# NVIDIA/cuopt

Measured on NVIDIA H100. Metric: pdlp_iterations_per_sec, higher is better.
Workload: dtype f64

## Files before the change

cuopt_b200/csrc/device_utils.cuh:

```cuda
#pragma once

#include "lp_problem.hpp"

#include <cuda_runtime.h>

#include <chrono>
#include <cstdio>
#include <cstdlib>
#include <mutex>
#include <string>
#include <vector>

namespace cuopt_b200 {

#define CUOPT_CUDA_TRY(call)                                                                              \
  do {                                                                                                    \
    cudaError_t err__ = (call);                                                                           \
    if (err__ != cudaSuccess) {                                                                           \
      cudaGetLastError();                                                                                 \
      throw ::cuopt_b200::lp_error(                                                                       \
        err__ == cudaErrorMemoryAllocation ? ::cuopt_b200::error_type_t::OutOfMemory                      \
                                           : ::cuopt_b200::error_type_t::RuntimeError,                    \
        std::string("CUDA error: ") + cudaGetErrorString(err__) + " at " + __FILE__ + ":" +               \
          std::to_string(__LINE__));                                                                      \
// ... 186 lines not shown
{
#pragma unroll
  for (int o = 16; o > 0; o >>= 1)
    v += __shfl_xor_sync(0xffffffffu, v, o);
  return v;
}
__device__ __forceinline__ double warp_max(double v)
{
#pragma unroll
  for (int o = 16; o > 0; o >>= 1)
    v = fmax(v, __shfl_xor_sync(0xffffffffu, v, o));
  return v;
}

template <bool IsMax = false>
__device__ __forceinline__ double block_reduce(double v, double* scratch)
{
  const int lane = threadIdx.x & 31, wid = threadIdx.x >> 5, nw = (blockDim.x + 31) >> 5;
  v = IsMax ? warp_max(v) : warp_sum(v);
  __syncthreads();
  if (lane == 0) scratch[wid] = v;
  __syncthreads();
  double r = (lane < nw) ? scratch[lane] : 0.0;
  r        = IsMax ? warp_max(r) : warp_sum(r);
  return r;
}

struct l2_policy_t {
  unsigned long long keep, stream;
};
__device__ __forceinline__ l2_policy_t make_l2_policies(int mode)
{
  l2_policy_t p;
  if (mode) {
    asm volatile("createpolicy.fractional.L2::evict_last.b64 %0, 1.0;" : "=l"(p.keep));
    asm volatile("createpolicy.fractional.L2::evict_first.b64 %0, 1.0;" : "=l"(p.stream));
  } else {
    asm volatile("createpolicy.fractional.L2::evict_normal.b64 %0, 1.0;" : "=l"(p.keep));
    p.stream = p.keep;
  }
  return p;
}
__device__ __forceinline__ double ld_l2(const double* p, unsigned long long policy)
{
  double v;
  asm volatile("ld.global.L1::no_allocate.L2::cache_hint.f64 %0, [%1], %2;" : "=d"(v) : "l"(p), "l"(policy));
  return v;
}
__device__ __forceinline__ void st_l2(double* p, double v, unsigned long long policy)
{
  asm volatile("st.global.L2::cache_hint.f64 [%0], %1, %2;" ::"l"(p), "d"(v), "l"(policy) : "memory");
}

__device__ __forceinline__ int ld_stream(const int* p) { return __ldcs(p); }
__device__ __forceinline__ double ld_stream(const double* p) { return __ldcs(p); }

}
```

cuopt_b200/csrc/pdlp_kernels.cuh:

```cuda
#pragma once

#include "device_utils.cuh"
#include "spmv_bicsr.cuh"

#include <math_constants.h>

namespace cuopt_b200 {

constexpr int EW_THREADS  = 256;
static __device__ int g_l2_hints = 1;

struct pdhg_ctl_t {
  double step_size, primal_weight, tau, sigma;
  double pending_weight;
  double sum_weights;
  double interaction, norm_dx2, norm_dy2;
  double reduction_exponent, growth_exponent, primal_smoothing, dual_smoothing;
  int parity;
  int pending_avg;
  int active;
  int valid;
  int k_pdhg;
  int attempts;
  int accepted;
// ... 144 lines not shown
                                                            int n,
                                                            double* __restrict__ xbuf0,
                                                            double* __restrict__ xbuf1,
                                                            const double* __restrict__ aty0,
                                                            const double* __restrict__ aty1,
                                                            const double* __restrict__ c,
                                                            const double* __restrict__ l,
                                                            const double* __restrict__ u,
                                                            double* __restrict__ sum_x,
                                                            double* __restrict__ xbar)
{
  if (!ctl->active) return;
  const int cur           = ctl->parity;
  const double* x         = cur ? xbuf1 : xbuf0;
  double* xn              = cur ? xbuf0 : xbuf1;
  const double* aty       = cur ? aty1 : aty0;
  const double tau        = ctl->tau;
  const bool pending      = ctl->pending_avg != 0;
  const double w          = ctl->pending_weight;
  const int stride        = gridDim.x * blockDim.x;
  const l2_policy_t pol   = make_l2_policies(g_l2_hints);
  for (int j = blockIdx.x * blockDim.x + threadIdx.x; j < n; j += stride) {
    const double xj = x[j];
    if (pending) sum_x[j] = sum_x[j] + w * xj;
    const double gradient = ld_stream(c + j) - aty[j];
    double next           = xj - (tau * gradient);
    next                  = fmax(fmin(next, ld_stream(u + j)), ld_stream(l + j));
    xn[j]                 = next;
    st_l2(xbar + j, next - xj + next, pol.keep);
  }
}

template <bool INIT, int NPRE, bool BCAST = false, int FMT = 0>
__global__ void __launch_bounds__(BICSR_THREADS, bicsr_min_ctas(NPRE)) k_dual_step(pdhg_ctl_t* __restrict__ ctl,
                                                                             bicsr_view_t A,
                                                                             const double* __restrict__ xbar,
                                                                             double* __restrict__ ybuf0,
                                                                             double* __restrict__ ybuf1,
                                                                             const double* __restrict__ lc,
                                                                             const double* __restrict__ uc,
                                                                             double* __restrict__ sum_y,
                                                                             double* __restrict__ part_dy2,
                                                                             const unsigned long long* xbar_flags,
                                                                             int n_xbar_flags,
                                                                             const double* __restrict__ t,
                                                                             peer_ptrs_t y_peers = peer_ptrs_t{},
                                                                             peer_flags_t flags = peer_flags_t{},
                                                                             int world = 1,
                                                                             int rank = 0,
                                                                             const int* __restrict__ send = nullptr,
                                                                             int send_stride = 0)
{
  if (!ctl->active) return;
  __shared__ double rows[BICSR_WARPS][BICSR_SLOTS];
  __shared__ double red[32];
  const unsigned long long epoch = (unsigned long long)ctl->attempts + 1ull;
  if (xbar_flags) peer_wait(xbar_flags, n_xbar_flags, (unsigned long long)ctl->attempts + 1ull);
  const int cur      = ctl->parity;
  const double* y    = cur ? ybuf1 : ybuf0;
  double* yn         = cur ? ybuf0 : ybuf1;
  const double sigma = ctl->sigma;
  const bool pending = ctl->pending_avg != 0;
  const double w     = ctl->pending_weight;
  double dy2         = 0.0;
  const l2_policy_t pol = make_l2_policies(g_l2_hints);
  struct payload_t {
    double y, lc, uc, sum, init;
  };
  auto pre_op = [&](int i) {
    payload_t p;
    p.y    = y[i];
    p.lc   = ld_stream(lc + i);
    p.uc   = ld_stream(uc + i);
    p.sum  = pending ? sum_y[i] : 0.0;
    p.init = INIT ? ld_l2(t + i, pol.stream) : 0.0;
    return p;
  };
  auto row_op = [&](int i, double s, const payload_t& p) {
    if (pending) sum_y[i] = p.sum + w * p.y;
    double next      = p.y - (sigma * s);
    const double low = next + sigma * p.lc;
    const double up  = next + sigma * p.uc;
    next             = fmax(low, fmin(up, 0.0));
    st_l2(yn + i, next, pol.keep);
    if constexpr (BCAST) {
#pragma unroll
      for (int r = 0; r < DIST_MAX_PEERS; ++r)
        if (r < world) {
          const int d = __ldg(send + (size_t)r * send_stride + i);
          if (d >= 0) y_peers.p[r][d] = next;
        }
    }
    const double d   = next - p.y;
    dy2 += d * d;
  };
  spmv_bicsr_rows<payload_t, INIT, NPRE, FMT>(A, xbar, rows[threadIdx.x >> 5], pre_op, row_op, pol.keep);
  const double tot = block_reduce(dy2, red);
  if (threadIdx.x == 0) part_dy2[blockIdx.x] = tot;
  if constexpr (BCAST) peer_signal_grid_done(&ctl->ticket[2], flags, world, DIST_FLAG_Y + rank, epoch, DIST_FLAG_Y_B + rank);
}

template <bool INIT, int NPRE, int FMT = 0>
__global__ void __launch_bounds__(BICSR_THREADS, bicsr_min_ctas(NPRE)) k_transpose_step(pdhg_ctl_t* __restrict__ ctl,
                                                                                  bicsr_view_t AT,
                                                                                  const double* __restrict__ ybuf0,
                                                                                  const double* __restrict__ ybuf1,
                                                                                  const double* __restrict__ xbuf0,
                                                                                  const double* __restrict__ xbuf1,
                                                                                  double* __restrict__ aty0,
                                                                                  double* __restrict__ aty1,
                                                                                  double* __restrict__ parts,
                                                                                  const double* __restrict__ part_dy2,
                                                                                  int n_part_dy2,
                                                                                  const double* __restrict__ t)
{
  if (!ctl->active) return;
  __shared__ double rows[BICSR_WARPS][BICSR_SLOTS];
  __shared__ double red[32];
  const int cur     = ctl->parity;
  const double* yn  = cur ? ybuf0 : ybuf1;
  const double* x   = cur ? xbuf1 : xbuf0;
  const double* xn  = cur ? xbuf0 : xbuf1;
  const double* aty = cur ? aty1 : aty0;
  double* atyn      = cur ? aty0 : aty1;
  double acc[2]     = {0.0, 0.0};
  const l2_policy_t pol = make_l2_policies(g_l2_hints);
  struct payload_t {
    double dx, aty, init;
  };
  auto pre_op = [&](int j) {
    payload_t p;
    p.dx   = ld_l2(xn + j, pol.stream) - ld_l2(x + j, pol.stream);
    p.aty  = ld_l2(aty + j, pol.stream);
    p.init = INIT ? ld_l2(t + j, pol.stream) : 0.0;
    return p;
  };
  auto row_op = [&](int j, double s, const payload_t& p) {
    st_l2(atyn + j, s, pol.stream);
    acc[0] += p.dx * (s - p.aty);
    acc[1] += p.dx * p.dx;
  };
  spmv_bicsr_rows<payload_t, INIT, NPRE, FMT>(AT, yn, rows[threadIdx.x >> 5], pre_op, row_op, pol.keep);

  if (!publish_and_elect<2>(acc, parts, &ctl->ticket[0], red)) return;
  const double interaction = gather_partials(parts, gridDim.x, red);
  const double dx2         = gather_partials(parts + gridDim.x, gridDim.x, red);
  const double dy2         = gather_partials(part_dy2, n_part_dy2, red);
  if (threadIdx.x != 0) return;

  pdhg_step_rule(ctl, interaction, dx2, dy2);
}

template <bool INIT, int NPRE>
__global__ void __launch_bounds__(BICSR_THREADS, bicsr_min_ctas(NPRE)) k_transpose_step_slice(pdhg_ctl_t* __restrict__ ctl,
                                                                                        bicsr_view_t AT,
                                                                                        const double* __restrict__ yfull,
                                                                                        const double* __restrict__ xbuf0,
                                                                                        const double* __restrict__ xbuf1,
                                                                                        double* __restrict__ aty0,
                                                                                        double* __restrict__ aty1,
                                                                                        double* __restrict__ parts,
                                                                                        const double* __restrict__ part_dy2,
                                                                                        int n_part_dy2,
                                                                                        const double* __restrict__ t,
                                                                                        const unsigned long long* wait_flags,
                                                                                        int n_wait,
                                                                                        peer_ptrs_t scal_peers,
                                                                                        peer_flags_t flags,
                                                                                        int world,
                                                                                        int rank)
{
  if (!ctl->active) return;
  __shared__ double rows[BICSR_WARPS][BICSR_SLOTS];
  __shared__ double red[32];
  const unsigned long long epoch = (unsigned long long)ctl->attempts + 1ull;
  if (wait_flags) peer_wait(wait_flags, n_wait, epoch);
  const int cur     = ctl->parity;
  const double* x   = cur ? xbuf1 : xbuf0;
  const double* xn  = cur ? xbuf0 : xbuf1;
  const double* aty = cur ? aty1 : aty0;
  double* atyn      = cur ? aty0 : aty1;
  double acc[2]     = {0.0, 0.0};
  const l2_policy_t pol = make_l2_policies(g_l2_hints);
  struct payload_t {
    double dx, aty, init;
  };
  auto pre_op = [&](int j) {
    payload_t p;
    p.dx   = ld_l2(xn + j, pol.stream) - ld_l2(x + j, pol.stream);
    p.aty  = ld_l2(aty + j, pol.stream);
    p.init = INIT ? ld_l2(t + j, pol.stream) : 0.0;
    return p;
  };
  auto row_op = [&](int j, double s, const payload_t& p) {
    st_l2(atyn + j, s, pol.stream);
    acc[0] += p.dx * (s - p.aty);
    acc[1] += p.dx * p.dx;
  };
  spmv_bicsr_rows<payload_t, INIT, NPRE>(AT, yfull, rows[threadIdx.x >> 5], pre_op, row_op, pol.keep);

  if (!publish_and_elect<2>(acc, parts, &ctl->ticket[0], red)) return;
  const double interaction = gather_partials(parts, gridDim.x, red);
  const double dx2         = gather_partials(parts + gridDim.x, gridDim.x, red);
  const double dy2         = gather_partials(part_dy2, n_part_dy2, red);
  if (threadIdx.x != 0) return;
#pragma unroll
  for (int r = 0; r < DIST_MAX_PEERS; ++r)
    if (r < world) {
      double* o = scal_peers.p[r];
      o[0]      = interaction;
      o[1]      = dx2;
      o[2]      = dy2;
    }
  __threadfence_system();
#pragma unroll
  for (int r = 0; r < DIST_MAX_PEERS; ++r)
    if (r < world) st_release_sys(flags.p[r] + DIST_FLAG_SCALARS + rank, epoch);
}

struct peer_csr_t {
  const int* off[DIST_MAX_PEERS];
  const int* idx[DIST_MAX_PEERS];
  const double* val[DIST_MAX_PEERS];
  int row0[DIST_MAX_PEERS];
};
__global__ void __launch_bounds__(EW_THREADS) k_slice_row_counts(int rows, int j0, peer_csr_t src, int world, int* __restrict__ cnt)
{
  const int stride = gridDim.x * blockDim.x;
  for (int j = blockIdx.x * blockDim.x + threadIdx.x; j <= rows; j += stride) {
    int c = 0;
    if (j < rows) {
#pragma unroll
      for (int g = 0; g < DIST_MAX_PEERS; ++g)
        if (g < world) c += src.off[g][j0 + j + 1] - src.off[g][j0 + j];
    }
    cnt[j] = c;
  }
}
__global__ void __launch_bounds__(EW_THREADS) k_slice_fill(int rows, int j0, peer_csr_t src, int world,
                                                           const int* __restrict__ soff, int* __restrict__ sidx,
                                                           double* __restrict__ sval)
{
  const int stride = gridDim.x * blockDim.x;
  for (int j = blockIdx.x * blockDim.x + threadIdx.x; j < rows; j += stride) {
    int p = soff[j];
#pragma unroll
    for (int g = 0; g < DIST_MAX_PEERS; ++g)
      if (g < world) {
        const int lo = src.off[g][j0 + j], hi = src.off[g][j0 + j + 1];
        for (int e = lo; e < hi; ++e, ++p) {
          sidx[p] = src.idx[g][e] + src.row0[g];
          sval[p] = src.val[g][e];
// ... 84 lines not shown
      int r = rank + 1 + d;
      if (r >= world) r -= world;
      int lo = 0, hi = 0;
      double* dst = peers.p[0];
#pragma unroll
      for (int q = 0; q < DIST_MAX_PEERS; ++q)
        if (q == r) {
          lo  = part ? plan.count_a[q] : 0;
          hi  = part ? plan.count[q] : plan.count_a[q];
          dst = peers.p[q];
        }
      if (hi <= lo) continue;
      const int* lst  = list + (size_t)r * stride;
      const int* slt  = slot + (size_t)r * stride;
      const int base  = __ldg(slt + __ldg(lst + lo));
      const int shift = base & 31;
      const int total = hi - lo + shift;
      for (int t0 = gtid; t0 < total; t0 += gstride * SEND_UNROLL) {
        int src[SEND_UNROLL];
        double val[SEND_UNROLL];
#pragma unroll
        for (int u = 0; u < SEND_UNROLL; ++u) {
          const int k = t0 + u * gstride - shift;
          src[u]      = (k >= 0 && k < hi - lo) ? __ldg(lst + lo + k) : -1;
        }
#pragma unroll
        for (int u = 0; u < SEND_UNROLL; ++u) val[u] = src[u] >= 0 ? v[src[u]] : 0.0;
#pragma unroll
        for (int u = 0; u < SEND_UNROLL; ++u)
          if (src[u] >= 0) dst[base + t0 + u * gstride - shift] = val[u];
      }
    }
    peer_signal_grid_done(tickets + part, flags, world, (part ? flag_b : flag_a) + rank, epoch);
    __syncthreads();
  }
}
__global__ void __launch_bounds__(EW_THREADS) k_remap_indices(int nnz, const int* __restrict__ idx_in, const int* __restrict__ pos,
                                                              int* __restrict__ idx_out)
{
  const int stride = gridDim.x * blockDim.x;
  for (int e = blockIdx.x * blockDim.x + threadIdx.x; e < nnz; e += stride) idx_out[e] = pos[idx_in[e]];
}

__global__ void __launch_bounds__(BICSR_THREADS, BICSR_MIN_CTAS) k_transpose_partial(const pdhg_ctl_t* __restrict__ ctl,
                                                                                     bicsr_view_t AT,
                                                                                     const double* __restrict__ ybuf0,
                                                                                     const double* __restrict__ ybuf1,
                                                                                     double* __restrict__ buf)
{
  if (!ctl->active) return;
  __shared__ double rows[BICSR_WARPS][BICSR_SLOTS];
  const double* yn = ctl->parity ? ybuf0 : ybuf1;
  struct payload_t {};
  auto pre_op = [&](int) { return payload_t{}; };
  auto row_op = [&](int j, double s, const payload_t&) { buf[j] = s; };
  spmv_bicsr_rows<payload_t>(AT, yn, rows[threadIdx.x >> 5], pre_op, row_op, make_l2_policies(g_l2_hints).keep);
}
__global__ void __launch_bounds__(EW_THREADS) k_sum_partials(const double* __restrict__ parts,
                                                             int count,
                                                             int n_quantities,
                                                             double* __restrict__ out)
{
  __shared__ double red[32];
  for (int q = 0; q < n_quantities; ++q) {
    double s = 0.0;
    for (int i = threadIdx.x; i < count; i += blockDim.x) s += parts[q * count + i];
    s = block_reduce(s, red);
    if (threadIdx.x == 0) out[q] = s;
  }
}

__global__ void __launch_bounds__(EW_THREADS) k_primal_step_bcast(pdhg_ctl_t* __restrict__ ctl,
                                                                  int nloc,
                                                                  double* __restrict__ xbuf0,
                                                                  double* __restrict__ xbuf1,
                                                                  const double* __restrict__ aty0,
                                                                  const double* __restrict__ aty1,
                                                                  const double* __restrict__ c,
                                                                  const double* __restrict__ l,
                                                                  const double* __restrict__ u,
                                                                  double* __restrict__ sum_x,
                                                                  peer_ptrs_t xbar_peers,
                                                                  peer_flags_t flags,
                                                                  int world,
                                                                  int rank,
                                                                  const int* __restrict__ send,
                                                                  int send_stride)
{
  if (!ctl->active) return;
  const unsigned long long epoch = (unsigned long long)ctl->attempts + 1ull;
  const int cur      = ctl->parity;
  const double* x    = cur ? xbuf1 : xbuf0;
  double* xn         = cur ? xbuf0 : xbuf1;
  const double* aty  = cur ? aty1 : aty0;
  const double tau   = ctl->tau;
  const bool pending = ctl->pending_avg != 0;
  const double w     = ctl->pending_weight;
  const int stride   = gridDim.x * blockDim.x;
  for (int j = blockIdx.x * blockDim.x + threadIdx.x; j < nloc; j += stride) {
    const double xj = x[j];
    if (pending) sum_x[j] = sum_x[j] + w * xj;
    const double gradient = ld_stream(c + j) - aty[j];
    double next           = xj - (tau * gradient);
    next                  = fmax(fmin(next, ld_stream(u + j)), ld_stream(l + j));
    xn[j]                 = next;
    const double xb       = next - xj + next;
#pragma unroll
    for (int r = 0; r < DIST_MAX_PEERS; ++r)
      if (r < world) {
// ... 21 lines not shown
  const int cur     = ctl->parity;
  const double* x   = cur ? xbuf1 : xbuf0;
  const double* xn  = cur ? xbuf0 : xbuf1;
  const double* aty = cur ? aty1 : aty0;
  double* atyn      = cur ? aty0 : aty1;
  double acc[2]     = {0.0, 0.0};
  const int stride  = gridDim.x * blockDim.x;
  for (int j = blockIdx.x * blockDim.x + threadIdx.x; j < nloc; j += stride) {
    double s = 0.0;
    s += __ldcg(src + j);
    atyn[j]        = s;
    const double d = xn[j] - x[j];
    acc[0] += d * (s - aty[j]);
    acc[1] += d * d;
  }
  if (!publish_and_elect<2>(acc, parts, &ctl->ticket[0], red)) return;
  const double interaction = gather_partials(parts, gridDim.x, red);
  const double dx2         = gather_partials(parts + gridDim.x, gridDim.x, red);
  const double dy2         = gather_partials(part_dy2, n_part_dy2, red);
  if (threadIdx.x != 0) return;
  scal[0] = interaction;
  scal[1] = dx2;
  scal[2] = dy2;
}

__global__ void k_step_rule_gather(pdhg_ctl_t* __restrict__ ctl, const double* __restrict__ scal, int n_src,
                                   const unsigned long long* wait_flags)
{
  if (!ctl->active) return;
  if (wait_flags) peer_wait(wait_flags, n_src, (unsigned long long)ctl->attempts + 1ull);
  if (threadIdx.x != 0) return;
  double interaction = 0.0, dx2 = 0.0, dy2 = 0.0;
  for (int g = 0; g < n_src; ++g) {
    interaction += __ldcg(scal + 4 * g + 0);
    dx2 += __ldcg(scal + 4 * g + 1);
    dy2 += __ldcg(scal + 4 * g + 2);
  }
  pdhg_step_rule(ctl, interaction, dx2, dy2);
}

template <int FMT = 0>
__global__ void __launch_bounds__(BICSR_THREADS, BICSR_MIN_CTAS) k_block_pass(const pdhg_ctl_t* __restrict__ ctl,
                                                                              bicsr_view_t Ab,
                                                                              const double* __restrict__ x0,
                                                                              const double* __restrict__ x1,
                                                                              int pick_candidate,
                                                                              double* __restrict__ t,
                                                                              int first,
                                                                              const unsigned long long* wait_flags,
                                                                              int n_wait)
{
  if (!ctl->active) return;
  __shared__ double rows[BICSR_WARPS][BICSR_SLOTS];
  if (wait_flags) peer_wait(wait_flags, n_wait, (unsigned long long)ctl->attempts + 1ull);
  const double* x       = pick_candidate ? (ctl->parity ? x0 : x1) : x0;
  const l2_policy_t pol = make_l2_policies(g_l2_hints);
  struct payload_t {
    double init;
  };
  auto pre_op = [&](int r) {
    payload_t p;
    p.init = first ? 0.0 : ld_l2(t + r, pol.stream);
    return p;
  };
  auto row_op = [&](int r, double s, const payload_t&) { st_l2(t + r, s, pol.stream); };
  spmv_bicsr_rows<payload_t, true, 1, FMT>(Ab, x, rows[threadIdx.x >> 5], pre_op, row_op, pol.keep);
}

__global__ void __launch_bounds__(EW_THREADS) k_flush_average(const pdhg_ctl_t* __restrict__ ctl,
                                                              int n,
                                                              const double* __restrict__ xbuf0,
                                                              const double* __restrict__ xbuf1,
                                                              double* __restrict__ sum_x,
                                                              int m,
                                                              const double* __restrict__ ybuf0,
                                                              const double* __restrict__ ybuf1,
                                                              double* __restrict__ sum_y)
{
  if (!ctl->pending_avg) return;
  const int cur    = ctl->parity;
  const double* x  = cur ? xbuf1 : xbuf0;
  const double* y  = cur ? ybuf1 : ybuf0;
  const double w   = ctl->pending_weight;
  const int stride = gridDim.x * blockDim.x;
  for (int j = blockIdx.x * blockDim.x + threadIdx.x; j < n; j += stride) sum_x[j] = sum_x[j] + w * x[j];
  for (int i = blockIdx.x * blockDim.x + threadIdx.x; i < m; i += stride) sum_y[i] = sum_y[i] + w * y[i];
}
__global__ void k_clear_pending(pdhg_ctl_t* ctl) { ctl->pending_avg = 0; }
__global__ void k_begin_batch(pdhg_ctl_t* ctl, int steps)
{
  ctl->target = ctl->accepted + steps;
  ctl->valid  = 0;
  ctl->active = steps > 0 ? 1 : 0;
}

__global__ void __launch_bounds__(BICSR_THREADS, BICSR_MIN_CTAS) k_spmv(bicsr_view_t A,
                                                                        const double* __restrict__ x,
                                                                        double* __restrict__ out)
{
  __shared__ double rows[BICSR_WARPS][BICSR_SLOTS];
  struct payload_t {};
  auto pre_op = [&](int) { return payload_t{}; };
  auto row_op = [&](int i, double s, const payload_t&) { out[i] = s; };
  spmv_bicsr_rows<payload_t>(A, x, rows[threadIdx.x >> 5], pre_op, row_op, make_l2_policies(g_l2_hints).keep);
}

template <int FMT = 0>
__global__ void __launch_bounds__(BICSR_THREADS, BICSR_MIN_CTAS) k_spmv_pair(bicsr_view_t M,
                                                                             const double* __restrict__ u,
                                                                             const double* __restrict__ v,
                                                                             double* __restrict__ out_u,
                                                                             double* __restrict__ out_v,
                                                                             int first)
{
  __shared__ double rows[2][BICSR_WARPS][BICSR_SLOTS];
  auto row_op = [&](int r, double su, double sv) {
    out_u[r] = first ? su : out_u[r] + su;
    out_v[r] = first ? sv : out_v[r] + sv;
  };
  const int w = threadIdx.x >> 5;
  spmv_bicsr_rows_pair<FMT>(M, u, v, rows[0][w], rows[1][w], row_op, make_l2_policies(g_l2_hints).keep);
}

__device__ __forceinline__ double bound_value_product(double value, double lower, double upper)
{
  double bound = 0.0;
  if (value > 0.0) bound = lower;
  else if (value < 0.0) bound = upper;
  return isfinite(bound) ? value * bound : 0.0;
}

__device__ __forceinline__ void eval_column(int j, const double (&s)[2], double cj, double lo, double hi,
                                            const double (&xv)[2], int reduced_cost_rule, double* __restrict__ rc_cur,
                                            double* __restrict__ rc_avg, double (&acc)[8])
{
  double* rcs[2] = {rc_cur, rc_avg};
#pragma unroll
  for (int v = 0; v < 2; ++v) {
    const double g     = cj - s[v];
    const double bound = g > 0.0 ? lo : hi;
    double rc;
    if (g == 0.0) rc = g;
    else if (reduced_cost_rule ? (fabs(xv[v] - bound) <= fabs(xv[v])) : isfinite(bound)) rc = g;
    else rc = 0.0;
    rcs[v][j]      = rc;
    const double r = g - rc;
    acc[v] += r * r;
    acc[2 + v] += bound_value_product(rc, lo, hi);
    acc[4 + v] += xv[v] * cj;
    acc[6 + v] += xv[v] * xv[v];
  }
}

__device__ __forceinline__ double gather_partials_max(const double* parts, int count, double* red)
{
  double s = 0.0;
  for (int i = threadIdx.x; i < count; i += blockDim.x) s = fmax(s, __ldcg(parts + i));
  return block_reduce<true>(s, red);
}

__device__ __forceinline__ void eval_finalize(pdhg_ctl_t* ctl, const double* parts, const double* parts_rows,
                                              int n_parts_rows, const eval_consts_t& k, eval_t* out, double* red,
                                              const double* max_cols = nullptr, const double* max_rows = nullptr,
                                              int n_max_rows = 0)
{
  double tot[14];
  for (int q = 0; q < 8; ++q) tot[q] = gather_partials(parts + q * gridDim.x, gridDim.x, red);
  for (int q = 0; q < 6; ++q) tot[8 + q] = gather_partials(parts_rows + q * n_parts_rows, n_parts_rows, red);
  double linf_p[2] = {0.0, 0.0}, linf_d[2] = {0.0, 0.0};
  if (k.per_constraint_residual && max_cols != nullptr && max_rows != nullptr) {
    for (int v = 0; v < 2; ++v) {
      linf_d[v] = gather_partials_max(max_cols + v * gridDim.x, gridDim.x, red);
      linf_p[v] = gather_partials_max(max_rows + v * n_max_rows, n_max_rows, red);
    }
// ... 496 lines not shown
```

cuopt_b200/csrc/spmv_bicsr.cuh:

```cuda
#pragma once

#include "device_utils.cuh"

namespace cuopt_b200 {

constexpr int BICSR_CH              = 8;
constexpr int BICSR_SLOTS           = 32 * BICSR_CH;
constexpr int BICSR_MAX_ROWS        = 256;
constexpr int BICSR_THREADS         = 256;
constexpr int BICSR_WARPS           = BICSR_THREADS / 32;
constexpr int BICSR_PAD             = 0x7fffffff;
constexpr unsigned short BICSR_EMPTY = 0xffff;
constexpr int BICSR_MIN_CTAS        = 4;
__host__ __device__ constexpr int bicsr_min_ctas(int npre) { return npre > 1 ? 3 : BICSR_MIN_CTAS; }

__host__ __device__ constexpr int bicsr_slot(int q) { return (q % BICSR_CH) * 32 + q / BICSR_CH; }

constexpr int BICSR_FMT_IDX3     = 1;
constexpr int BICSR_FMT_MASK     = 2;
constexpr int BICSR_IDX3_MAX_WIDTH = 1 << 21;
constexpr unsigned BICSR_HI_PAD  = 0x40u;
constexpr unsigned BICSR_HI_END  = 0x80u;

struct bicsr_view_t {
  const int2* desc;
  const unsigned short* row_slot;
  const int* idx;
  const double* val;
  int n_std, n_blk;
  const int* off;
  const int* cidx;
  const double* cval;
  const unsigned short* lo16;
  const unsigned long long* hi8;
  const unsigned* mask;
  int col0;
};

template <int FMT>
struct bicsr_cols_t {
  int c[BICSR_CH];
};
template <>
struct bicsr_cols_t<BICSR_FMT_IDX3> {
  uint4 lo;
  unsigned long long hi;
};
template <>
struct bicsr_cols_t<BICSR_FMT_IDX3 | BICSR_FMT_MASK> : bicsr_cols_t<BICSR_FMT_IDX3> {};
template <>
struct bicsr_cols_t<BICSR_FMT_MASK> : bicsr_cols_t<0> {};

template <int FMT>
__device__ __forceinline__ void bicsr_load_cols(const bicsr_view_t& A, int b, int lane, bicsr_cols_t<FMT>& w)
{
// ... 36 lines not shown
}

struct bicsr_mask_cursor_t {
  unsigned mw;
  int base;
  __device__ __forceinline__ int next(int q, int lane)
  {
    const unsigned m = __shfl_sync(0xffffffffu, mw, q);
    const int ord    = ((m >> lane) & 1u) ? base + __popc(m & ((1u << lane) - 1u)) : -1;
    base += __popc(m);
    return ord;
  }
};

__device__ __forceinline__ int bicsr_ends_before(unsigned ends, int lane)
{
  const unsigned cnt = __popc(ends), lt = (1u << lane) - 1u;
  int before         = 0;
#pragma unroll
  for (int j = 0; j < 4; ++j) before += __popc(__ballot_sync(0xffffffffu, (cnt >> j) & 1u) & lt) << j;
  return before;
}

template <bool MASK = false>
__device__ __forceinline__ void bicsr_block_row_sums(const double (&a)[BICSR_CH], const double (&g)[BICSR_CH], unsigned ends,
                                                     int lane, double* rsw, int before = 0)
{
  constexpr unsigned FULL = 0xffffffffu;
  double s = 0.0, head = 0.0;
  const int kf = ends ? __ffs(ends) - 1 : -1;
  int ord      = before;
#pragma unroll
  for (int k = 0; k < BICSR_CH; ++k) {
    s = __dadd_rn(s, __dmul_rn(a[k], g[k]));
    const bool e = (ends >> k) & 1u;
    if (e && k != kf) rsw[MASK ? ord : k * 32 + lane] = s;
    if constexpr (MASK) ord += e;
    head = (k == kf) ? s : head;
    s    = e ? 0.0 : s;
  }
  double tail  = s;
  double carry = __shfl_up_sync(FULL, tail, 1);
  if (lane == 0) carry = 0.0;
  unsigned pending = __ballot_sync(FULL, kf < 0);
  while (pending) {
    if (kf < 0) tail = carry + s;
    carry = __shfl_up_sync(FULL, tail, 1);
    if (lane == 0) carry = 0.0;
    pending &= pending << 1;
  }
  if (kf >= 0) rsw[MASK ? before : kf * 32 + lane] = carry + head;
}

template <typename P, bool INIT = false, int NPRE = 1, int FMT = 0, typename PreOp, typename RowOp>
__device__ __forceinline__ void spmv_bicsr_rows(const bicsr_view_t& A,
                                                const double* __restrict__ x,
                                                double* rsw,
                                                PreOp& pre_op,
                                                RowOp& row_op,
                                                unsigned long long gather_policy)
{
  constexpr bool MASK     = (FMT & BICSR_FMT_MASK) != 0;
  const int lane          = threadIdx.x & 31;
  const int gwarp         = blockIdx.x * BICSR_WARPS + (threadIdx.x >> 5);
  const int nwarps        = gridDim.x * BICSR_WARPS;
  const double* xg        = bicsr_gather_base<FMT>(A, x);
  bicsr_cols_t<FMT> c;
  if (gwarp < A.n_std) bicsr_load_cols<FMT>(A, gwarp, lane, c);
  for (int b = gwarp; b < A.n_std; b += nwarps) {
    const int2 d  = __ldg(A.desc + b);
    const int r0 = d.x, r1 = d.y;
    P pl[NPRE];
    unsigned short slot[NPRE];
    bicsr_mask_cursor_t mc{0u, 0};
#pragma unroll
    for (int q = 0; q < NPRE; ++q) {
      slot[q] = BICSR_EMPTY;
      if (r0 + lane + 32 * q < r1) {
        pl[q] = pre_op(r0 + lane + 32 * q);
        if constexpr (!MASK) slot[q] = __ldg(A.row_slot + r0 + lane + 32 * q);
      }
    }
    const size_t base = (size_t)b * BICSR_SLOTS + lane;
    double a[BICSR_CH], g[BICSR_CH];
#pragma unroll
    for (int k = 0; k < BICSR_CH; ++k) a[k] = ld_stream(A.val + base + k * 32);
#pragma unroll
    for (int k = 0; k < BICSR_CH; ++k) {
      const int col = bicsr_col<FMT>(c, k);
      g[k]          = col >= 0 ? ld_l2(xg + col, gather_policy) : 0.0;
    }
    if constexpr (MASK) mc.mw = lane < 8 ? __ldg(A.mask + (size_t)b * 8 + lane) : 0u;
    const unsigned ends = bicsr_ends<FMT>(c);
    if (b + nwarps < A.n_std) bicsr_load_cols<FMT>(A, b + nwarps, lane, c);
    bicsr_block_row_sums<MASK>(a, g, ends, lane, rsw, MASK ? bicsr_ends_before(ends, lane) : 0);
    __syncwarp();
#pragma unroll
    for (int q = 0; q < NPRE; ++q) {
      int src = slot[q] != BICSR_EMPTY ? (int)slot[q] : -1;
      if constexpr (MASK) src = mc.next(q, lane);
      if (r0 + lane + 32 * q < r1) {
        double sum = src >= 0 ? rsw[src] : 0.0;
        if constexpr (INIT) sum = pl[q].init + sum;
        row_op(r0 + lane + 32 * q, sum, pl[q]);
      }
    }
    for (int q = NPRE; 32 * q < r1 - r0; ++q) {
      const int r = r0 + 32 * q + lane;
      int src     = -1;
      if constexpr (MASK) src = mc.next(q, lane);
      if (r < r1) {
        const P p2 = pre_op(r);
        if constexpr (!MASK) {
          const unsigned short s2 = __ldg(A.row_slot + r);
          src                     = s2 != BICSR_EMPTY ? (int)s2 : -1;
        }
        double sum = src >= 0 ? rsw[src] : 0.0;
        if constexpr (INIT) sum = p2.init + sum;
        row_op(r, sum, p2);
      }
    }
    __syncwarp();
  }
  for (int b = A.n_std + gwarp; b < A.n_blk; b += nwarps) {
    const int row = __ldg(A.desc + b).x;
    const int lo = __ldg(A.off + row), hi = __ldg(A.off + row + 1);
    P pl;
    if (lane == 0) pl = pre_op(row);
    double acc = 0.0;
    for (int e = lo + lane; e < hi; e += 32) acc += ld_stream(A.cval + e) * ld_l2(x + ld_stream(A.cidx + e), gather_policy);
    acc = warp_sum(acc);
    if (lane == 0) {
      if constexpr (INIT) acc = pl.init + acc;
      row_op(row, acc, pl);
    }
  }
}

template <int FMT = 0, typename RowOp>
__device__ __forceinline__ void spmv_bicsr_rows_pair(const bicsr_view_t& A,
                                                     const double* __restrict__ u,
                                                     const double* __restrict__ v,
                                                     double* rsw_u,
                                                     double* rsw_v,
                                                     RowOp& row_op,
                                                     unsigned long long gather_policy)
{
  constexpr bool MASK = (FMT & BICSR_FMT_MASK) != 0;
  const int lane   = threadIdx.x & 31;
  const int gwarp  = blockIdx.x * BICSR_WARPS + (threadIdx.x >> 5);
  const int nwarps = gridDim.x * BICSR_WARPS;
  const double* ug = bicsr_gather_base<FMT>(A, u);
  const double* vg = bicsr_gather_base<FMT>(A, v);
  for (int b = gwarp; b < A.n_std; b += nwarps) {
    const int2 d      = __ldg(A.desc + b);
    const size_t base = (size_t)b * BICSR_SLOTS + lane;
    bicsr_cols_t<FMT> c;
    double a[BICSR_CH], gu[BICSR_CH], gv[BICSR_CH];
    bicsr_load_cols<FMT>(A, b, lane, c);
    bicsr_mask_cursor_t mc{0u, 0};
#pragma unroll
    for (int k = 0; k < BICSR_CH; ++k) a[k] = ld_stream(A.val + base + k * 32);
#pragma unroll
    for (int k = 0; k < BICSR_CH; ++k) {
      const int col = bicsr_col<FMT>(c, k);
      gu[k]         = col >= 0 ? ld_l2(ug + col, gather_policy) : 0.0;
      gv[k]         = col >= 0 ? ld_l2(vg + col, gather_policy) : 0.0;
    }
    const unsigned ends = bicsr_ends<FMT>(c);
    const int before    = MASK ? bicsr_ends_before(ends, lane) : 0;
    bicsr_block_row_sums<MASK>(a, gu, ends, lane, rsw_u, before);
    bicsr_block_row_sums<MASK>(a, gv, ends, lane, rsw_v, before);
    if constexpr (MASK) mc.mw = lane < 8 ? __ldg(A.mask + (size_t)b * 8 + lane) : 0u;
    __syncwarp();
    for (int q = 0; 32 * q < d.y - d.x; ++q) {
      const int r = d.x + 32 * q + lane;
      int s       = -1;
      if constexpr (MASK) s = mc.next(q, lane);
      if (r < d.y) {
        if constexpr (!MASK) {
          const unsigned short s2 = __ldg(A.row_slot + r);
          s                       = s2 != BICSR_EMPTY ? (int)s2 : -1;
        }
        row_op(r, s >= 0 ? rsw_u[s] : 0.0, s >= 0 ? rsw_v[s] : 0.0);
      }
    }
    __syncwarp();
  }
  for (int b = A.n_std + gwarp; b < A.n_blk; b += nwarps) {
    const int row = __ldg(A.desc + b).x;
    const int lo = __ldg(A.off + row), hi = __ldg(A.off + row + 1);
    double acc_u = 0.0, acc_v = 0.0;
    for (int e = lo + lane; e < hi; e += 32) {
      const double a = ld_stream(A.cval + e);
      const int col  = ld_stream(A.cidx + e);
      acc_u += a * ld_l2(u + col, gather_policy);
      acc_v += a * ld_l2(v + col, gather_policy);
    }
    acc_u = warp_sum(acc_u);
    acc_v = warp_sum(acc_v);
    if (lane == 0) row_op(row, acc_u, acc_v);
  }
}

__global__ void __launch_bounds__(256) k_bicsr_fill(int n_std,
                                                    const int2* __restrict__ desc,
                                                    const int* __restrict__ off,
                                                    const int* __restrict__ idx,
                                                    const double* __restrict__ val,
                                                    int* __restrict__ bidx,
                                                    double* __restrict__ bval,
                                                    unsigned short* __restrict__ row_slot)
{
  const int lane = threadIdx.x & 31, wpb = blockDim.x >> 5;
  for (int b = blockIdx.x * wpb + (threadIdx.x >> 5); b < n_std; b += gridDim.x * wpb) {
    const int2 d      = desc[b];
    const int lo      = off[d.x];
    const size_t base = (size_t)b * BICSR_SLOTS;
    const int cnt = off[d.y] - lo;
#pragma unroll
    for (int k = 0; k < BICSR_CH; ++k) {
      const int q                = BICSR_CH * lane + k;
      bidx[base + k * 32 + lane] = q < cnt ? idx[lo + q] : BICSR_PAD;
      if (bval) bval[base + k * 32 + lane] = q < cnt ? val[lo + q] : 0.0;
    }
    __syncwarp();
    for (int r = d.x + lane; r < d.y; r += 32) {
      const int p0 = off[r], p1 = off[r + 1];
      unsigned short slot = BICSR_EMPTY;
      if (p1 > p0) {
        slot = (unsigned short)bicsr_slot(p1 - 1 - lo);
        bidx[base + slot] |= (int)0x80000000u;
      }
      row_slot[r] = slot;
    }
    __syncwarp();
  }
}
__global__ void __launch_bounds__(256) k_bicsr_fill_values(int n_std,
                                                           const int2* __restrict__ desc,
                                                           const int* __restrict__ off,
                                                           const double* __restrict__ val,
                                                           double* __restrict__ bval)
{
  const int lane = threadIdx.x & 31, wpb = blockDim.x >> 5;
  for (int b = blockIdx.x * wpb + (threadIdx.x >> 5); b < n_std; b += gridDim.x * wpb) {
    const int2 d      = desc[b];
    const int lo      = off[d.x];
    const int cnt     = off[d.y] - lo;
    const size_t base = (size_t)b * BICSR_SLOTS;
#pragma unroll
    for (int k = 0; k < BICSR_CH; ++k) {
      const int q                = BICSR_CH * lane + k;
      bval[base + k * 32 + lane] = q < cnt ? val[lo + q] : 0.0;
// ... 55 lines not shown
```

Before: 399.3.

## Prefetch per-row payload vectors into shared memory with cp.async in BiCSR SpMV

Replaces the per-row pre_op loads of payload vectors (y, bounds, sums, init) with a generic payload descriptor. Rows beyond the prefetched groups are now staged asynchronously into a per-warp shared-memory buffer via cp.async, issued before the gather and block row-sum work. The goal is to overlap payload memory latency with the SpMV gather instead of loading serially in the row epilogue. In exchange it adds extra shared memory per block, which may reduce occupancy, and a wait_group barrier on each stage chunk. The AT kernels keep direct loads.

```diff
diff --git a/cuopt_b200/csrc/device_utils.cuh b/cuopt_b200/csrc/device_utils.cuh
--- a/cuopt_b200/csrc/device_utils.cuh
+++ b/cuopt_b200/csrc/device_utils.cuh
@@ -262,6 +262,17 @@
   asm volatile("st.global.L2::cache_hint.f64 [%0], %1, %2;" ::"l"(p), "d"(v), "l"(policy) : "memory");
 }
 
+__device__ __forceinline__ void cp_async_8(double* dst, const double* src, int src_bytes, unsigned long long policy)
+{
+  asm volatile("cp.async.ca.shared.global.L2::cache_hint [%0], [%1], 8, %2, %3;" ::"r"((unsigned)__cvta_generic_to_shared(dst)),
+               "l"(src), "r"(src_bytes), "l"(policy)
+               : "memory");
+}
+__device__ __forceinline__ void cp_async_wait()
+{
+  asm volatile("cp.async.commit_group;\n\tcp.async.wait_group 0;" ::: "memory");
+}
+
 __device__ __forceinline__ int ld_stream(const int* p) { return __ldcs(p); }
 __device__ __forceinline__ double ld_stream(const double* p) { return __ldcs(p); }
 
diff --git a/cuopt_b200/csrc/pdlp_kernels.cuh b/cuopt_b200/csrc/pdlp_kernels.cuh
--- a/cuopt_b200/csrc/pdlp_kernels.cuh
+++ b/cuopt_b200/csrc/pdlp_kernels.cuh
@@ -220,7 +220,9 @@
                                                                              int send_stride = 0)
 {
   if (!ctl->active) return;
+  constexpr int NARR = INIT ? 5 : 4;
   __shared__ double rows[BICSR_WARPS][BICSR_SLOTS];
+  __shared__ double stage[BICSR_WARPS][bicsr_stage_doubles(NARR, NPRE, BICSR_STAGE_BYTES)];
   __shared__ double red[32];
   const unsigned long long epoch = (unsigned long long)ctl->attempts + 1ull;
   if (xbar_flags) peer_wait(xbar_flags, n_xbar_flags, (unsigned long long)ctl->attempts + 1ull);
@@ -235,15 +237,13 @@
   struct payload_t {
     double y, lc, uc, sum, init;
   };
-  auto pre_op = [&](int i) {
-    payload_t p;
-    p.y    = y[i];
-    p.lc   = ld_stream(lc + i);
-    p.uc   = ld_stream(uc + i);
-    p.sum  = pending ? sum_y[i] : 0.0;
-    p.init = INIT ? ld_l2(t + i, pol.stream) : 0.0;
-    return p;
-  };
+  bicsr_payload_t<NARR> pay;
+  pay.a[0] = y;
+  pay.a[1] = lc;
+  pay.a[2] = uc;
+  pay.a[3] = pending ? sum_y : nullptr;
+  if constexpr (INIT) pay.a[NARR - 1] = t;
+  auto make_op = [&](const double (&v)[NARR]) { return payload_t{v[0], v[1], v[2], v[3], INIT ? v[NARR - 1] : 0.0}; };
   auto row_op = [&](int i, double s, const payload_t& p) {
     if (pending) sum_y[i] = p.sum + w * p.y;
     double next      = p.y - (sigma * s);
@@ -262,7 +262,7 @@
     const double d   = next - p.y;
     dy2 += d * d;
   };
-  spmv_bicsr_rows<payload_t, INIT, NPRE, FMT>(A, xbar, rows[threadIdx.x >> 5], pre_op, row_op, pol.keep);
+  spmv_bicsr_rows<INIT, NPRE, FMT>(A, xbar, rows[threadIdx.x >> 5], pay, stage[threadIdx.x >> 5], make_op, row_op, pol);
   const double tot = block_reduce(dy2, red);
   if (threadIdx.x == 0) part_dy2[blockIdx.x] = tot;
   if constexpr (BCAST) peer_signal_grid_done(&ctl->ticket[2], flags, world, DIST_FLAG_Y + rank, epoch, DIST_FLAG_Y_B + rank);
@@ -283,6 +283,7 @@
                                                                                   const double* __restrict__ t)
 {
   if (!ctl->active) return;
+  constexpr int NARR = INIT ? 4 : 3;
   __shared__ double rows[BICSR_WARPS][BICSR_SLOTS];
   __shared__ double red[32];
   const int cur     = ctl->parity;
@@ -296,19 +297,18 @@
   struct payload_t {
     double dx, aty, init;
   };
-  auto pre_op = [&](int j) {
-    payload_t p;
-    p.dx   = ld_l2(xn + j, pol.stream) - ld_l2(x + j, pol.stream);
-    p.aty  = ld_l2(aty + j, pol.stream);
-    p.init = INIT ? ld_l2(t + j, pol.stream) : 0.0;
-    return p;
-  };
+  bicsr_payload_t<NARR> pay;
+  pay.a[0] = xn;
+  pay.a[1] = x;
+  pay.a[2] = aty;
+  if constexpr (INIT) pay.a[NARR - 1] = t;
+  auto make_op = [&](const double (&v)[NARR]) { return payload_t{v[0] - v[1], v[2], INIT ? v[NARR - 1] : 0.0}; };
   auto row_op = [&](int j, double s, const payload_t& p) {
     st_l2(atyn + j, s, pol.stream);
     acc[0] += p.dx * (s - p.aty);
     acc[1] += p.dx * p.dx;
   };
-  spmv_bicsr_rows<payload_t, INIT, NPRE, FMT>(AT, yn, rows[threadIdx.x >> 5], pre_op, row_op, pol.keep);
+  spmv_bicsr_rows<INIT, NPRE, FMT, false>(AT, yn, rows[threadIdx.x >> 5], pay, nullptr, make_op, row_op, pol);
 
   if (!publish_and_elect<2>(acc, parts, &ctl->ticket[0], red)) return;
   const double interaction = gather_partials(parts, gridDim.x, red);
@@ -339,6 +339,7 @@
                                                                                         int rank)
 {
   if (!ctl->active) return;
+  constexpr int NARR = INIT ? 4 : 3;
   __shared__ double rows[BICSR_WARPS][BICSR_SLOTS];
   __shared__ double red[32];
   const unsigned long long epoch = (unsigned long long)ctl->attempts + 1ull;
@@ -353,19 +354,18 @@
   struct payload_t {
     double dx, aty, init;
   };
-  auto pre_op = [&](int j) {
-    payload_t p;
-    p.dx   = ld_l2(xn + j, pol.stream) - ld_l2(x + j, pol.stream);
-    p.aty  = ld_l2(aty + j, pol.stream);
-    p.init = INIT ? ld_l2(t + j, pol.stream) : 0.0;
-    return p;
-  };
+  bicsr_payload_t<NARR> pay;
+  pay.a[0] = xn;
+  pay.a[1] = x;
+  pay.a[2] = aty;
+  if constexpr (INIT) pay.a[NARR - 1] = t;
+  auto make_op = [&](const double (&v)[NARR]) { return payload_t{v[0] - v[1], v[2], INIT ? v[NARR - 1] : 0.0}; };
   auto row_op = [&](int j, double s, const payload_t& p) {
     st_l2(atyn + j, s, pol.stream);
     acc[0] += p.dx * (s - p.aty);
     acc[1] += p.dx * p.dx;
   };
-  spmv_bicsr_rows<payload_t, INIT, NPRE>(AT, yfull, rows[threadIdx.x >> 5], pre_op, row_op, pol.keep);
+  spmv_bicsr_rows<INIT, NPRE, 0, false>(AT, yfull, rows[threadIdx.x >> 5], pay, nullptr, make_op, row_op, pol);
 
   if (!publish_and_elect<2>(acc, parts, &ctl->ticket[0], red)) return;
   const double interaction = gather_partials(parts, gridDim.x, red);
@@ -556,9 +556,9 @@
   __shared__ double rows[BICSR_WARPS][BICSR_SLOTS];
   const double* yn = ctl->parity ? ybuf0 : ybuf1;
   struct payload_t {};
-  auto pre_op = [&](int) { return payload_t{}; };
-  auto row_op = [&](int j, double s, const payload_t&) { buf[j] = s; };
-  spmv_bicsr_rows<payload_t>(AT, yn, rows[threadIdx.x >> 5], pre_op, row_op, make_l2_policies(g_l2_hints).keep);
+  auto make_op = [](const double (&)[1]) { return payload_t{}; };
+  auto row_op  = [&](int j, double s, const payload_t&) { buf[j] = s; };
+  spmv_bicsr_rows(AT, yn, rows[threadIdx.x >> 5], bicsr_payload_t<0>{}, nullptr, make_op, row_op, make_l2_policies(g_l2_hints));
 }
 __global__ void __launch_bounds__(EW_THREADS) k_sum_partials(const double* __restrict__ parts,
                                                              int count,
@@ -686,19 +686,17 @@
 {
   if (!ctl->active) return;
   __shared__ double rows[BICSR_WARPS][BICSR_SLOTS];
+  __shared__ double stage[BICSR_WARPS][bicsr_stage_doubles(1, 1, BICSR_STAGE_BYTES)];
   if (wait_flags) peer_wait(wait_flags, n_wait, (unsigned long long)ctl->attempts + 1ull);
   const double* x       = pick_candidate ? (ctl->parity ? x0 : x1) : x0;
   const l2_policy_t pol = make_l2_policies(g_l2_hints);
   struct payload_t {
     double init;
   };
-  auto pre_op = [&](int r) {
-    payload_t p;
-    p.init = first ? 0.0 : ld_l2(t + r, pol.stream);
-    return p;
-  };
-  auto row_op = [&](int r, double s, const payload_t&) { st_l2(t + r, s, pol.stream); };
-  spmv_bicsr_rows<payload_t, true, 1, FMT>(Ab, x, rows[threadIdx.x >> 5], pre_op, row_op, pol.keep);
+  const bicsr_payload_t<1> pay{{first ? nullptr : t}};
+  auto make_op = [](const double (&v)[1]) { return payload_t{v[0]}; };
+  auto row_op  = [&](int r, double s, const payload_t&) { st_l2(t + r, s, pol.stream); };
+  spmv_bicsr_rows<true, 1, FMT>(Ab, x, rows[threadIdx.x >> 5], pay, stage[threadIdx.x >> 5], make_op, row_op, pol);
 }
 
 __global__ void __launch_bounds__(EW_THREADS) k_flush_average(const pdhg_ctl_t* __restrict__ ctl,
@@ -734,9 +732,9 @@
 {
   __shared__ double rows[BICSR_WARPS][BICSR_SLOTS];
   struct payload_t {};
-  auto pre_op = [&](int) { return payload_t{}; };
-  auto row_op = [&](int i, double s, const payload_t&) { out[i] = s; };
-  spmv_bicsr_rows<payload_t>(A, x, rows[threadIdx.x >> 5], pre_op, row_op, make_l2_policies(g_l2_hints).keep);
+  auto make_op = [](const double (&)[1]) { return payload_t{}; };
+  auto row_op  = [&](int i, double s, const payload_t&) { out[i] = s; };
+  spmv_bicsr_rows(A, x, rows[threadIdx.x >> 5], bicsr_payload_t<0>{}, nullptr, make_op, row_op, make_l2_policies(g_l2_hints));
 }
 
 template <int FMT = 0>
@@ -748,12 +746,15 @@
                                                                              int first)
 {
   __shared__ double rows[2][BICSR_WARPS][BICSR_SLOTS];
-  auto row_op = [&](int r, double su, double sv) {
+  struct payload_t {};
+  auto make_op = [](const double (&)[1]) { return payload_t{}; };
+  auto row_op = [&](int r, double su, double sv, const payload_t&) {
     out_u[r] = first ? su : out_u[r] + su;
     out_v[r] = first ? sv : out_v[r] + sv;
   };
   const int w = threadIdx.x >> 5;
-  spmv_bicsr_rows_pair<FMT>(M, u, v, rows[0][w], rows[1][w], row_op, make_l2_policies(g_l2_hints).keep);
+  spmv_bicsr_rows_pair<FMT>(M, u, v, rows[0][w], rows[1][w], bicsr_payload_t<0>{}, nullptr, make_op, row_op,
+                            make_l2_policies(g_l2_hints));
 }
 
 __device__ __forceinline__ double bound_value_product(double value, double lower, double upper)
diff --git a/cuopt_b200/csrc/spmv_bicsr.cuh b/cuopt_b200/csrc/spmv_bicsr.cuh
--- a/cuopt_b200/csrc/spmv_bicsr.cuh
+++ b/cuopt_b200/csrc/spmv_bicsr.cuh
@@ -1,6 +1,8 @@
 #pragma once
 
 #include "device_utils.cuh"
+
+#include <utility>
 
 namespace cuopt_b200 {
 
@@ -143,24 +145,74 @@
   if (kf >= 0) rsw[MASK ? before : kf * 32 + lane] = carry + head;
 }
 
-template <typename P, bool INIT = false, int NPRE = 1, int FMT = 0, typename PreOp, typename RowOp>
+template <int N>
+struct bicsr_payload_t {
+  const double* a[N > 0 ? N : 1];
+};
+
+constexpr int BICSR_STAGE_BYTES      = 3840;
+constexpr int BICSR_PAIR_STAGE_BYTES = 2048;
+__host__ __device__ constexpr int bicsr_stage_groups(int narr, int npre, int bytes)
+{
+  return (narr == 0 || bytes / (narr * 8 * 32) >= BICSR_MAX_ROWS / 32 - npre) ? BICSR_MAX_ROWS / 32 - npre
+                                                                               : bytes / (narr * 8 * 32);
+}
+__host__ __device__ constexpr int bicsr_stage_doubles(int narr, int npre, int bytes)
+{
+  return narr * 32 * bicsr_stage_groups(narr, npre, bytes);
+}
+
+template <int N, int G>
+__device__ __forceinline__ void bicsr_stage_issue(const bicsr_payload_t<N>& pay, double* stage, int r0, int r1, int q0,
+                                                  int lane, unsigned long long policy)
+{
+#pragma unroll
+  for (int q = 0; q < G; ++q) {
+    if (32 * (q0 + q) >= r1 - r0) break;
+    const int r = r0 + 32 * (q0 + q) + lane;
+#pragma unroll
+    for (int k = 0; k < N; ++k)
+      if (pay.a[k]) cp_async_8(stage + (k * G + q) * 32 + lane, pay.a[k] + (r < r1 ? r : r0), r < r1 ? 8 : 0, policy);
+  }
+}
+template <int N, int G>
+__device__ __forceinline__ void bicsr_stage_read(const bicsr_payload_t<N>& pay, const double* stage, int q, int lane,
+                                                 double (&v)[N > 0 ? N : 1])
+{
+#pragma unroll
+  for (int k = 0; k < N; ++k) v[k] = pay.a[k] ? stage[(k * G + q) * 32 + lane] : 0.0;
+}
+
+template <bool INIT = false, int NPRE = 1, int FMT = 0, bool STAGE = true, int N, typename MakeOp, typename RowOp>
 __device__ __forceinline__ void spmv_bicsr_rows(const bicsr_view_t& A,
                                                 const double* __restrict__ x,
                                                 double* rsw,
-                                                PreOp& pre_op,
+                                                const bicsr_payload_t<N>& pay,
+                                                double* stage,
+                                                MakeOp& make_op,
                                                 RowOp& row_op,
-                                                unsigned long long gather_policy)
+                                                l2_policy_t policy)
 {
   constexpr bool MASK     = (FMT & BICSR_FMT_MASK) != 0;
+  constexpr int G         = STAGE ? bicsr_stage_groups(N, NPRE, BICSR_STAGE_BYTES) : BICSR_MAX_ROWS / 32 - NPRE;
+  using V                 = double[N > 0 ? N : 1];
+  using P                 = decltype(make_op(std::declval<const V&>()));
   const int lane          = threadIdx.x & 31;
   const int gwarp         = blockIdx.x * BICSR_WARPS + (threadIdx.x >> 5);
   const int nwarps        = gridDim.x * BICSR_WARPS;
   const double* xg        = bicsr_gather_base<FMT>(A, x);
+  auto load = [&](int r) {
+    V v = {};
+#pragma unroll
+    for (int k = 0; k < N; ++k) v[k] = pay.a[k] ? ld_l2(pay.a[k] + r, policy.stream) : 0.0;
+    return make_op(v);
+  };
   bicsr_cols_t<FMT> c;
   if (gwarp < A.n_std) bicsr_load_cols<FMT>(A, gwarp, lane, c);
   for (int b = gwarp; b < A.n_std; b += nwarps) {
     const int2 d  = __ldg(A.desc + b);
     const int r0 = d.x, r1 = d.y;
+    if constexpr (STAGE) bicsr_stage_issue<N, G>(pay, stage, r0, r1, NPRE, lane, policy.stream);
     P pl[NPRE];
     unsigned short slot[NPRE];
     bicsr_mask_cursor_t mc{0u, 0};
@@ -168,7 +220,7 @@
     for (int q = 0; q < NPRE; ++q) {
       slot[q] = BICSR_EMPTY;
       if (r0 + lane + 32 * q < r1) {
-        pl[q] = pre_op(r0 + lane + 32 * q);
+        pl[q] = load(r0 + lane + 32 * q);
         if constexpr (!MASK) slot[q] = __ldg(A.row_slot + r0 + lane + 32 * q);
       }
     }
@@ -179,7 +231,7 @@
 #pragma unroll
     for (int k = 0; k < BICSR_CH; ++k) {
       const int col = bicsr_col<FMT>(c, k);
-      g[k]          = col >= 0 ? ld_l2(xg + col, gather_policy) : 0.0;
+      g[k]          = col >= 0 ? ld_l2(xg + col, policy.keep) : 0.0;
     }
     if constexpr (MASK) mc.mw = lane < 8 ? __ldg(A.mask + (size_t)b * 8 + lane) : 0u;
     const unsigned ends = bicsr_ends<FMT>(c);
@@ -196,19 +248,32 @@
         row_op(r0 + lane + 32 * q, sum, pl[q]);
       }
     }
-    for (int q = NPRE; 32 * q < r1 - r0; ++q) {
-      const int r = r0 + 32 * q + lane;
-      int src     = -1;
-      if constexpr (MASK) src = mc.next(q, lane);
-      if (r < r1) {
-        const P p2 = pre_op(r);
-        if constexpr (!MASK) {
-          const unsigned short s2 = __ldg(A.row_slot + r);
-          src                     = s2 != BICSR_EMPTY ? (int)s2 : -1;
+    for (int q0 = NPRE; 32 * q0 < r1 - r0; q0 += G) {
+      if constexpr (STAGE && N > 0) {
+        if (q0 > NPRE) bicsr_stage_issue<N, G>(pay, stage, r0, r1, q0, lane, policy.stream);
+        cp_async_wait();
+      }
+      for (int q = q0; q < q0 + G && 32 * q < r1 - r0; ++q) {
+        const int r = r0 + 32 * q + lane;
+        int src     = -1;
+        if constexpr (MASK) src = mc.next(q, lane);
+        if (r < r1) {
+          P p2;
+          if constexpr (STAGE) {
+            V v = {};
+            bicsr_stage_read<N, G>(pay, stage, q - q0, lane, v);
+            p2 = make_op(v);
+          } else {
+            p2 = load(r);
+          }
+          if constexpr (!MASK) {
+            const unsigned short s2 = __ldg(A.row_slot + r);
+            src                     = s2 != BICSR_EMPTY ? (int)s2 : -1;
+          }
+          double sum = src >= 0 ? rsw[src] : 0.0;
+          if constexpr (INIT) sum = p2.init + sum;
+          row_op(r, sum, p2);
         }
-        double sum = src >= 0 ? rsw[src] : 0.0;
-        if constexpr (INIT) sum = p2.init + sum;
-        row_op(r, sum, p2);
       }
     }
     __syncwarp();
@@ -217,9 +282,9 @@
     const int row = __ldg(A.desc + b).x;
     const int lo = __ldg(A.off + row), hi = __ldg(A.off + row + 1);
     P pl;
-    if (lane == 0) pl = pre_op(row);
+    if (lane == 0) pl = load(row);
     double acc = 0.0;
-    for (int e = lo + lane; e < hi; e += 32) acc += ld_stream(A.cval + e) * ld_l2(x + ld_stream(A.cidx + e), gather_policy);
+    for (int e = lo + lane; e < hi; e += 32) acc += ld_stream(A.cval + e) * ld_l2(x + ld_stream(A.cidx + e), policy.keep);
     acc = warp_sum(acc);
     if (lane == 0) {
       if constexpr (INIT) acc = pl.init + acc;
@@ -228,16 +293,21 @@
   }
 }
 
-template <int FMT = 0, typename RowOp>
+template <int FMT = 0, int N, typename MakeOp, typename RowOp>
 __device__ __forceinline__ void spmv_bicsr_rows_pair(const bicsr_view_t& A,
                                                      const double* __restrict__ u,
                                                      const double* __restrict__ v,
                                                      double* rsw_u,
                                                      double* rsw_v,
+                                                     const bicsr_payload_t<N>& pay,
+                                                     double* stage,
+                                                     MakeOp& make_op,
                                                      RowOp& row_op,
-                                                     unsigned long long gather_policy)
+                                                     l2_policy_t policy)
 {
   constexpr bool MASK = (FMT & BICSR_FMT_MASK) != 0;
+  constexpr int G     = bicsr_stage_groups(N, 0, BICSR_PAIR_STAGE_BYTES);
+  using V             = double[N > 0 ? N : 1];
   const int lane   = threadIdx.x & 31;
   const int gwarp  = blockIdx.x * BICSR_WARPS + (threadIdx.x >> 5);
   const int nwarps = gridDim.x * BICSR_WARPS;
@@ -246,6 +316,7 @@
   for (int b = gwarp; b < A.n_std; b += nwarps) {
     const int2 d      = __ldg(A.desc + b);
     const size_t base = (size_t)b * BICSR_SLOTS + lane;
+    bicsr_stage_issue<N, G>(pay, stage, d.x, d.y, 0, lane, policy.stream);
     bicsr_cols_t<FMT> c;
     double a[BICSR_CH], gu[BICSR_CH], gv[BICSR_CH];
     bicsr_load_cols<FMT>(A, b, lane, c);
@@ -255,8 +326,8 @@
 #pragma unroll
     for (int k = 0; k < BICSR_CH; ++k) {
       const int col = bicsr_col<FMT>(c, k);
-      gu[k]         = col >= 0 ? ld_l2(ug + col, gather_policy) : 0.0;
-      gv[k]         = col >= 0 ? ld_l2(vg + col, gather_policy) : 0.0;
+      gu[k]         = col >= 0 ? ld_l2(ug + col, policy.keep) : 0.0;
+      gv[k]         = col >= 0 ? ld_l2(vg + col, policy.keep) : 0.0;
     }
     const unsigned ends = bicsr_ends<FMT>(c);
     const int before    = MASK ? bicsr_ends_before(ends, lane) : 0;
@@ -264,16 +335,22 @@
     bicsr_block_row_sums<MASK>(a, gv, ends, lane, rsw_v, before);
     if constexpr (MASK) mc.mw = lane < 8 ? __ldg(A.mask + (size_t)b * 8 + lane) : 0u;
     __syncwarp();
-    for (int q = 0; 32 * q < d.y - d.x; ++q) {
-      const int r = d.x + 32 * q + lane;
-      int s       = -1;
-      if constexpr (MASK) s = mc.next(q, lane);
-      if (r < d.y) {
-        if constexpr (!MASK) {
-          const unsigned short s2 = __ldg(A.row_slot + r);
-          s                       = s2 != BICSR_EMPTY ? (int)s2 : -1;
+    for (int q0 = 0; 32 * q0 < d.y - d.x; q0 += G) {
+      if (q0 > 0) bicsr_stage_issue<N, G>(pay, stage, d.x, d.y, q0, lane, policy.stream);
+      if constexpr (N > 0) cp_async_wait();
+      for (int q = q0; q < q0 + G && 32 * q < d.y - d.x; ++q) {
+        const int r = d.x + 32 * q + lane;
+        int s       = -1;
+        if constexpr (MASK) s = mc.next(q, lane);
+        if (r < d.y) {
+          V w = {};
+          bicsr_stage_read<N, G>(pay, stage, q - q0, lane, w);
+          if constexpr (!MASK) {
+            const unsigned short s2 = __ldg(A.row_slot + r);
+            s                       = s2 != BICSR_EMPTY ? (int)s2 : -1;
+          }
+          row_op(r, s >= 0 ? rsw_u[s] : 0.0, s >= 0 ? rsw_v[s] : 0.0, make_op(w));
         }
-        row_op(r, s >= 0 ? rsw_u[s] : 0.0, s >= 0 ? rsw_v[s] : 0.0);
       }
     }
     __syncwarp();
@@ -285,12 +362,17 @@
     for (int e = lo + lane; e < hi; e += 32) {
       const double a = ld_stream(A.cval + e);
       const int col  = ld_stream(A.cidx + e);
-      acc_u += a * ld_l2(u + col, gather_policy);
-      acc_v += a * ld_l2(v + col, gather_policy);
+      acc_u += a * ld_l2(u + col, policy.keep);
+      acc_v += a * ld_l2(v + col, policy.keep);
     }
     acc_u = warp_sum(acc_u);
     acc_v = warp_sum(acc_v);
-    if (lane == 0) row_op(row, acc_u, acc_v);
+    if (lane == 0) {
+      V w = {};
+#pragma unroll
+      for (int k = 0; k < N; ++k) w[k] = pay.a[k] ? ld_l2(pay.a[k] + row, policy.stream) : 0.0;
+      row_op(row, acc_u, acc_v, make_op(w));
+    }
   }
 }
 
```

Result: no change. 400.2, median of 6 (+0.2%).
